# kocurvik/mdrp

Hardware: AMD Instinct MI355X
Metric: image-pairs/sec (2000 corrs, 10k RANSAC iters) (higher is better)
Workload: dtype f64

## Files before the change

mdrp_amd/build.py:

```python
import hashlib
import os
import re
import shutil
import subprocess

HERE = os.path.dirname(os.path.abspath(__file__))
SRC = os.path.join(HERE, "csrc", "mdrp_capi.hip")
SRC_TU = os.path.join(HERE, "csrc", "mdrp_tu.hip")
TU_GROUPS = (1, 2, 3)
DEPS = [SRC, SRC_TU, os.path.join(HERE, "csrc", "mdrp_kernels.h"), os.path.join(HERE, "csrc", "mdrp_math.h"),
        os.path.join(HERE, "csrc", "mdrp_classic.h"), os.path.join(HERE, "csrc", "mdrp_classic_math.h"),
        os.path.join(HERE, "csrc", "mdrp_logtab.h"), os.path.join(HERE, "csrc", "mdrp_instances.h"),
        os.path.join(HERE, "..", "include", "mdrp.h")]
OUT = os.path.join(HERE, "libmdrp_hip.so")
_MARK = b"MDRP_SRC_HASH="
FLAGS = ["-O3", "-std=c++17", "--offload-arch=gfx950", "-fPIC", "-shared", "-ffp-contract=fast", "-no-hip-rt"]


def hipcc():
    for c in (shutil.which("hipcc"), "/opt/rocm/bin/hipcc"):
        if c and os.path.exists(c):
            return c
    raise RuntimeError("hipcc not found")


def source_hash():
    h = hashlib.sha256()
    h.update(" ".join(FLAGS).encode())
    for d in DEPS:
        h.update(os.path.basename(d).encode() + b"\0")
        with open(d, "rb") as f:
            h.update(f.read())
    return h.hexdigest()[:16]


def built_hash(path=OUT):
    try:
        with open(path, "rb") as f:
            m = re.search(_MARK + rb"([0-9a-f]{16})", f.read())
        return m.group(1).decode() if m else None
    except OSError:
        return None


def up_to_date():
    return built_hash() == source_hash()


def build(force=False, verbose=False, defines=(), out=OUT, extra_flags=(), single=None):
    if not force and not defines and not extra_flags and out == OUT and up_to_date():
        return out
    if single is None:
        single = bool(defines) or bool(extra_flags)
    common = [*FLAGS, *extra_flags, f'-DMDRP_SRC_HASH="{source_hash()}"', *[f"-D{d}" for d in defines]]
    if verbose:
        common.insert(0, "-Rpass-analysis=kernel-resource-usage")
    if single:
        subprocess.check_call([hipcc(), *common, SRC, "-o", out + ".tmp"])
        os.replace(out + ".tmp", out)
        return out
    import tempfile
    from concurrent.futures import ThreadPoolExecutor
# ... 26 lines not shown
```

mdrp_amd/csrc/mdrp_capi.hip:

```cpp
#include "../../include/mdrp.h"
#include "mdrp_kernels.h"
#include "mdrp_classic.h"
#ifdef MDRP_SPLIT_TU
#define MDRP_INST extern
#include "mdrp_instances.h"
namespace mdrp {
MDRP_INSTANCES_FINAL_64
MDRP_INSTANCES_FINAL_256
MDRP_INSTANCES_CLASSIC
}
#endif

#include <algorithm>
#include <cmath>
#include <cstdio>
#include <cstdlib>
#include <cstddef>
#include <cstring>
#include <functional>
#include <map>
#include <mutex>
#include <string>
#include <vector>

using namespace mdrp;

static_assert(sizeof(mdrp_model) == sizeof(Model), "model layout");
static_assert(sizeof(mdrp_camera) == sizeof(CamDev), "camera layout");
static_assert(sizeof(mdrp_result) == sizeof(ResultDev), "result layout");

namespace {

thread_local std::string g_err;

#define HIPCHK(expr)                                                                                       \
    do {                                                                                                   \
        hipError_t e_ = (expr);                                                                            \
        if (e_ != hipSuccess) {                                                                            \
            char buf_[512];                                                                                \
            snprintf(buf_, sizeof buf_, "%s failed: %s (%s:%d)", #expr, hipGetErrorString(e_), __FILE__, __LINE__); \
            g_err = buf_;                                                                                  \
            return MDRP_ERR_HIP;                                                                           \
        }                                                                                                  \
    } while (0)

struct DevBuf {
    void *p = nullptr;
    size_t cap = 0;
    int ensure(size_t bytes) {
        if (bytes <= cap) return MDRP_OK;
        if (p) { (void)hipFree(p); p = nullptr; cap = 0; }
        size_t want = bytes + bytes / 8 + 256;
        hipError_t e = hipMalloc(&p, want);
        if (e != hipSuccess) { g_err = std::string("hipMalloc failed: ") + hipGetErrorString(e); p = nullptr; return MDRP_ERR_HIP; }
        cap = want;
        return MDRP_OK;
    }
    void release() { if (p) (void)hipFree(p); p = nullptr; cap = 0; }
    template <typename T> T *as() const { return reinterpret_cast<T *>(p); }
};

struct Progress {
// ... 432 lines not shown
            int rc_;
            if ((rc_ = get_events(h, &e0, &e1, 0))) return rc_;
            unsigned long long *cstats = reinterpret_cast<unsigned long long *>(cnt + 6);
            {
                hipEvent_t c0, c1;
                if ((rc_ = get_events(h, &c0, &c1, 1))) return rc_;
                const bool two_phase = !(it0 == 0 && c == 0);
                unsigned long long *cand_stat = h->cand_stat.as<unsigned long long>() + 2 * (size_t)p0;
                uint32_t *tags_u = tags_sc;
                int32_t *und_part = reinterpret_cast<int32_t *>((odd ? h->tags_s : h->tags2_s).as<uint32_t>() + so), *und_cnt = h->und_count.as<int32_t>() + 2 * (size_t)p0;
                const uint4 *rfrag_p = h->rfrag.as<uint4>() + (size_t)p0 * groups_max * 64;
                hipLaunchKernelGGL(k_count_plan, dim3(1), dim3(PLAN_THREADS), 0, s, pc, st_p, mcount_c, 2, CNT_WG_MODELS, h->cplan.as<int32_t>(),
                                   surv1, (const int32_t *)nullptr, two_phase ? und_cnt : (int32_t *)nullptr);
                const dim3 cgrid((unsigned)pc * (unsigned)((len * mps + CNT_WG_MODELS - 1) / CNT_WG_MODELS));
                HIPCHK(hipEventRecord(c0, s));
                MDRP_SWEEP_DISPATCH(k_count, kind, cgrid, dim3(CNT_THREADS), 0, s, r, st_p, rfrag_p, models_p,
                                    tags_c, mcount_c, h->cplan.as<int32_t>(), tags_v, surv1, cstats, (int32_t *)nullptr, (const int32_t *)nullptr,
                                    1, tags_u, und_part, und_cnt, (const int32_t *)nullptr, cand_stat);
                if (two_phase) {
                    hipLaunchKernelGGL(k_count_plan, dim3(1), dim3(PLAN_THREADS), 0, s, pc, st_p, und_cnt, 2, CNT_WG_MODELS, h->cplan.as<int32_t>(),
                                       (int32_t *)nullptr, (const int32_t *)nullptr, (int32_t *)nullptr);
                    MDRP_SWEEP_DISPATCH(k_count, kind, cgrid, dim3(CNT_THREADS), 0, s, r, st_p, rfrag_p, models_p,
                                        tags_u, und_cnt, h->cplan.as<int32_t>(), tags_v, surv1, cstats, (int32_t *)nullptr, (const int32_t *)nullptr,
                                        2, (uint32_t *)nullptr, (int32_t *)nullptr, (int32_t *)nullptr, und_part, cand_stat);
                    h->count_launches++;
                }
                HIPCHK(hipEventRecord(c1, s));
                h->count_launches++;
            }
            const uint32_t *surv_tags = tags_v;
            const int32_t *surv_cnt = surv1;
            if (use_bound && batch_call > 16 && !(it0 == 0 && c == 0)) {
                hipLaunchKernelGGL(k_count_plan, dim3(1), dim3(PLAN_THREADS), 0, s, pc, st_p, surv1, 1, BND_THREADS, h->cplan.as<int32_t>(), surv2, (const int32_t *)nullptr);
                const dim3 bgrid((unsigned)pc * (unsigned)((len * mps + BND_THREADS - 1) / BND_THREADS));
                unsigned long long *bstats = reinterpret_cast<unsigned long long *>(cnt + 12);
                hipEvent_t b0, b1;
                if ((rc_ = get_events(h, &b0, &b1, 4))) return rc_;
                HIPCHK(hipEventRecord(b0, s));
                MDRP_SWEEP_DISPATCH(k_bound, kind, bgrid, dim3(BND_THREADS), 0, s, r, st_p, pts_p, models_p, tags_v, surv1, h->cplan.as<int32_t>(), tags_c, surv2, bstats);
                HIPCHK(hipEventRecord(b1, s));
                surv_tags = tags_c; surv_cnt = surv2;
            }
            int32_t *plan = h->plan.as<int32_t>(), *totals = plan + 2 * (size_t)batch + 2;
            if (batch_call <= SCORE_WAVE_MAX_PAIRS) {
                hipLaunchKernelGGL(k_count_plan, dim3(1), dim3(PLAN_THREADS), 0, s, pc, st_p, surv_cnt, 1, SCW_THREADS / 64, plan, (int32_t *)nullptr, (const int32_t *)nullptr, (int32_t *)nullptr);
                hipLaunchKernelGGL(k_sort_tags, dim3(pc), dim3(256), 0, s, r, st_p, mcount_c, surv_cnt, surv_tags, tags_sc);
                HIPCHK(hipEventRecord(e0, s));
                const long long ub = (long long)pc * ((len * mps + SCW_THREADS / 64 - 1) / (SCW_THREADS / 64));
                const dim3 grid((unsigned)std::min<long long>(ub, (long long)h->num_cu * 32));
                MDRP_SWEEP_DISPATCH(k_score_w, kind, grid, dim3(SCW_THREADS), 0, s, r, st_p, pts_p, models_p, tags_sc, mcount_c,
                                    h->slot_score.as<double>() + so, h->slot_inl.as<int32_t>() + so, plan);
            } else {
                hipLaunchKernelGGL(k_sort_tags, dim3(pc), dim3(256), 0, s, r, st_p, mcount_c, surv_cnt, surv_tags, tags_sc);
                hipLaunchKernelGGL(k_plan, dim3(1), dim3(PLAN_THREADS), 0, s, pc, mcount_c, plan, totals);
                HIPCHK(hipEventRecord(e0, s));
                const dim3 grid((unsigned)pc * (unsigned)((len * mps + SCORE_THREADS - 1) / SCORE_THREADS));
                MDRP_SWEEP_DISPATCH(k_score, kind, grid, dim3(SCORE_THREADS), tile_bytes, s, r, st_p, pts_p, models_p, tags_sc, mcount_c,
                                    h->slot_score.as<double>() + so, h->slot_inl.as<int32_t>() + so, plan, totals);
            }
            HIPCHK(hipEventRecord(e1, s));
            h->sweep_launches++;
            Trigger *trig_p = h->triggers.as<Trigger>() + (size_t)p0 * trig_cap;
            unsigned long long *scan_stats = reinterpret_cast<unsigned long long *>(cnt + 10);
#define MDRP_SCAN(M, I) hipLaunchKernelGGL((k_scan<M, I>), dim3(pc), dim3(64), 0, s, r, st_p, h->slot_score.as<double>() + so, h->slot_inl.as<int32_t>() + so, trig_p, trig_cap, mcount_c, scan_stats)
            if (mps == 16) MDRP_SCAN(16, 1);
            else if (mps == 12) MDRP_SCAN(12, 1);
            else if (len >= 1024) MDRP_SCAN(4, 4);
            else MDRP_SCAN(4, 1);
#undef MDRP_SCAN
            return MDRP_OK;
        };
        bool solved1 = false;
        int swept0 = 0;
        if (host && it0 == 0) {
            const bool sliced = piped && n_chunks >= 2 && batch >= 2 * HOST_SLICE_PAIRS;
            const int sl = sliced ? HOST_SLICE_PAIRS : batch;
            for (int p0 = 0; p0 < batch; p0 += sl) {
                const int pc = std::min(sl, batch - p0);
                const size_t o2 = (size_t)2 * p0 * n_max, o1 = (size_t)p0 * n_max, n2 = sizeof(double) * 2 * (size_t)pc * n_max, n1 = sizeof(double) * (size_t)pc * n_max;
                hipStream_t cs = sliced ? h->copy_stream : s;
                HIPCHK(hipMemcpyAsync(const_cast<double *>(x1) + o2, host->x1 + o2, n2, hipMemcpyHostToDevice, cs));
                HIPCHK(hipMemcpyAsync(const_cast<double *>(x2) + o2, host->x2 + o2, n2, hipMemcpyHostToDevice, cs));
                if (host->d1 && host->d2) {
                    HIPCHK(hipMemcpyAsync(const_cast<double *>(d1) + o1, host->d1 + o1, n1, hipMemcpyHostToDevice, cs));
                    HIPCHK(hipMemcpyAsync(const_cast<double *>(d2) + o1, host->d2 + o1, n1, hipMemcpyHostToDevice, cs));
                }
                if (!sliced) { launch_prep(p0, pc, s); break; }
                HIPCHK(hipEventRecord(h->ev_copied, cs)); HIPCHK(hipStreamWaitEvent(aux, h->ev_copied, 0));
                if (p0 == 0) HIPCHK(hipStreamWaitEvent(aux, h->ev_tables, 0));
                launch_prep(p0, pc, aux);
                HIPCHK(hipEventRecord(h->ev_prepped, aux));
                if ((rc = issue_solve(1, aux, p0, pc))) return rc;
                const bool last = p0 + sl >= batch, last_but_one = !last && p0 + 2 * sl >= batch;
                if (last_but_one || last) HIPCHK(hipStreamWaitEvent(s, h->ev_prepped, 0));
                if (last_but_one) { swept0 = p0 + pc; if ((rc = issue_solve(0, s, 0, swept0)) || (rc = sweep_chunk(0, 0, swept0))) return rc; }
                if (last) { if ((rc = issue_solve(0, s, swept0, batch - swept0)) || (rc = sweep_chunk(0, swept0, batch - swept0))) return rc; swept0 = batch; }
            }
            if (sliced) { HIPCHK(hipEventRecord(h->ev_solved[1], aux)); solved1 = true; }
        }
        if (swept0 < batch && (rc = issue_solve(0, s, 0, batch))) return rc;
        if (piped) HIPCHK(hipEventRecord(h->ev_solved[0], s));
        for (int c = 0; c < n_chunks; ++c) {
            rp.chunk_len = (int)lens[c]; rp.chunk_off = offs[c];
            if (c == 0 && swept0 >= batch) {
                if (piped) HIPCHK(hipEventRecord(h->ev_scanned[0], s));
                continue;
            }
            if (piped && c + 1 < n_chunks && !(c == 0 && solved1)) {
                HIPCHK(hipStreamWaitEvent(aux, c == 0 ? h->ev_solved[0] : h->ev_scanned[c - 1], 0));
                if ((rc = issue_solve(c + 1, aux, 0, batch))) return rc;
                HIPCHK(hipEventRecord(h->ev_solved[c + 1], aux));
// ... 452 lines not shown
    HIPCHK(hipMemcpyAsync(out, h->unit_e.p, sizeof(Model) * M * count, hipMemcpyDeviceToHost, s));
    HIPCHK(hipMemcpyAsync(n_out, h->unit_f.p, sizeof(int32_t) * count, hipMemcpyDeviceToHost, s));
    HIPCHK(hipStreamSynchronize(s));
    return MDRP_OK;
}

int mdrp_score_models(mdrp_handle *h, int kind, int mem_space, const mdrp_model *models, int num_models, const double *x1,
                      const double *x2, int n, double sq_threshold, double *scores, int32_t *counts) {
    if (!h || num_models < 0 || n < 0 || kind < 0 || kind > 5 || !scores || !counts) { g_err = "invalid argument"; return MDRP_ERR_INVALID; }
    if (num_models == 0) return MDRP_OK;
    MDRP_ENTER(h);
    hipStream_t s = h->stream;
    const int chunk = (num_models + 3) / 4;
    const size_t slots = (size_t)chunk * 4;
    int rc;
    if ((rc = h->pts.ensure(sizeof(double) * PT_STRIDE * std::max(n, 1))) || (rc = h->st.ensure(sizeof(PairState))) ||
        (rc = h->models.ensure(sizeof(Model) * slots)) || (rc = h->slot_score.ensure(sizeof(double) * slots)) ||
        (rc = h->slot_inl.ensure(sizeof(int32_t) * slots)) || (rc = h->tags.ensure(sizeof(uint32_t) * slots)) ||
        (rc = h->model_count.ensure(2 * sizeof(int32_t))))
        return rc;
    const double *x1d = x1, *x2d = x2;
    const Model *md = reinterpret_cast<const Model *>(models);
    if (mem_space == MDRP_MEM_HOST) {
        if ((rc = h->in_x1.ensure(sizeof(double) * 2 * std::max(n, 1))) || (rc = h->in_x2.ensure(sizeof(double) * 2 * std::max(n, 1)))) return rc;
        HIPCHK(hipMemcpyAsync(h->in_x1.p, x1, sizeof(double) * 2 * n, hipMemcpyHostToDevice, s));
        HIPCHK(hipMemcpyAsync(h->in_x2.p, x2, sizeof(double) * 2 * n, hipMemcpyHostToDevice, s));
        HIPCHK(hipMemcpyAsync(h->models.p, models, sizeof(Model) * num_models, hipMemcpyHostToDevice, s));
        x1d = h->in_x1.as<double>(); x2d = h->in_x2.as<double>();
        md = h->models.as<Model>();
    } else {
        HIPCHK(hipMemcpyAsync(h->models.p, models, sizeof(Model) * num_models, hipMemcpyDeviceToDevice, s));
        md = h->models.as<Model>();
    }
    std::vector<uint32_t> tags(num_models);
    for (int i = 0; i < num_models; ++i) tags[i] = (uint32_t)i;
    HIPCHK(hipMemcpyAsync(h->tags.p, tags.data(), sizeof(uint32_t) * num_models, hipMemcpyHostToDevice, s));
    const int32_t counts2[2] = {num_models, 0};
    HIPCHK(hipMemcpyAsync(h->model_count.p, counts2, 2 * sizeof(int32_t), hipMemcpyHostToDevice, s));
    PairState ps;
    std::memset(&ps, 0, sizeof ps);
    ps.n = n; ps.active = 1; ps.sq_thr = sq_threshold; ps.eps = std::sqrt(sq_threshold);
    ps.best_min_score = DBL_MAX;
    HIPCHK(hipMemcpyAsync(h->st.p, &ps, sizeof ps, hipMemcpyHostToDevice, s));
    hipLaunchKernelGGL(k_pack_unit, dim3((n + 255) / 256 + 1), dim3(256), 0, s, n, x1d, x2d, (const double *)nullptr,
                       (const double *)nullptr, h->pts.as<double>(), (double *)nullptr);
    hipLaunchKernelGGL(k_box_unit, dim3(1), dim3(256), 0, s, n, h->pts.as<double>(), h->st.as<PairState>());
    RunParams rp;
    std::memset(&rp, 0, sizeof rp);
    rp.kind = kind; rp.batch = 1; rp.n_max = std::max(n, 1); rp.chunk_len = chunk; rp.chunk_off = 0; rp.slot_stride = chunk * 4; rp.super_len = chunk;
    rp.mps = 4; rp.sample_sz = 3;
    const size_t tile_bytes = SCORE_TILE_BYTES;
    if ((rc = h->plan.ensure(sizeof(int32_t) * 8))) return rc;
    int32_t *plan = h->plan.as<int32_t>(), *totals = plan + 4;
    hipLaunchKernelGGL(k_plan, dim3(1), dim3(PLAN_THREADS), 0, s, 1, h->model_count.as<int32_t>(), plan, totals);
    const dim3 grid((unsigned)std::min(h->num_cu * 4, (num_models + SCORE_THREADS - 1) / SCORE_THREADS));
    h->ev_used = 0; h->sweep_launches = 1; h->sweep_evals = (int64_t)num_models * n;
    hipEvent_t e0, e1;
    if ((rc = get_events(h, &e0, &e1))) return rc;
    HIPCHK(hipEventRecord(e0, s));
    MDRP_SWEEP_DISPATCH(k_score, kind, grid, dim3(SCORE_THREADS), tile_bytes, s, rp, h->st.as<PairState>(), h->pts.as<double>(), md,
                        h->tags.as<uint32_t>(), h->model_count.as<int32_t>(), h->slot_score.as<double>(), h->slot_inl.as<int32_t>(), plan, totals);
    HIPCHK(hipEventRecord(e1, s));
    HIPCHK(hipGetLastError());
    const hipMemcpyKind back = mem_space == MDRP_MEM_HOST ? hipMemcpyDeviceToHost : hipMemcpyDeviceToDevice;
    HIPCHK(hipMemcpyAsync(scores, h->slot_score.p, sizeof(double) * num_models, back, s));
    HIPCHK(hipMemcpyAsync(counts, h->slot_inl.p, sizeof(int32_t) * num_models, back, s));
    return finish_timing(h);
}

int mdrp_count_candidates(mdrp_handle *h, int kind, const mdrp_model *models, int num_models, const double *x1, const double *x2,
                          int n, double sq_threshold, int32_t *candidates) {
    if (!h || num_models < 0 || n < 0 || kind < 0 || kind > 5 || !candidates || !models) { g_err = "invalid argument"; return MDRP_ERR_INVALID; }
    if (num_models == 0) return MDRP_OK;
    MDRP_ENTER(h);
    hipStream_t s = h->stream;
    const int nn = std::max(n, 1);
    const size_t slots = (size_t)num_models;
    int rc;
    if ((rc = h->pts.ensure(sizeof(double) * PT_STRIDE * nn)) || (rc = h->st.ensure(sizeof(PairState))) ||
        (rc = h->models.ensure(sizeof(Model) * slots)) || (rc = h->slot_inl.ensure(sizeof(int32_t) * slots)) ||
        (rc = h->tags.ensure(sizeof(uint32_t) * slots)) || (rc = h->tags_v.ensure(sizeof(uint32_t) * slots)) ||
        (rc = h->model_count.ensure(2 * sizeof(int32_t))) || (rc = h->surv_count.ensure(sizeof(int32_t))) ||
        (rc = h->cplan.ensure(2 * sizeof(int32_t))) || (rc = h->rfrag.ensure((size_t)((nn + 15) / 16) * 1024)) ||
        (rc = h->unit_f.ensure(sizeof(int32_t) * slots)) || (rc = h->in_x1.ensure(sizeof(double) * 2 * nn)) ||
        (rc = h->in_x2.ensure(sizeof(double) * 2 * nn)))
        return rc;
    HIPCHK(hipMemcpyAsync(h->in_x1.p, x1, sizeof(double) * 2 * n, hipMemcpyHostToDevice, s));
    HIPCHK(hipMemcpyAsync(h->in_x2.p, x2, sizeof(double) * 2 * n, hipMemcpyHostToDevice, s));
    HIPCHK(hipMemcpyAsync(h->models.p, models, sizeof(Model) * num_models, hipMemcpyHostToDevice, s));
    std::vector<uint32_t> tags(num_models);
    for (int i = 0; i < num_models; ++i) tags[i] = (uint32_t)i;
    HIPCHK(hipMemcpyAsync(h->tags.p, tags.data(), sizeof(uint32_t) * num_models, hipMemcpyHostToDevice, s));
    const int32_t counts2[2] = {num_models, 0};
    HIPCHK(hipMemcpyAsync(h->model_count.p, counts2, 2 * sizeof(int32_t), hipMemcpyHostToDevice, s));
    HIPCHK(hipMemsetAsync(h->surv_count.p, 0, sizeof(int32_t), s));
    PairState ps;
    std::memset(&ps, 0, sizeof ps);
    ps.n = n; ps.active = 1; ps.sq_thr = sq_threshold; ps.eps = std::sqrt(sq_threshold);
    ps.best_min_score = DBL_MAX;
    HIPCHK(hipMemcpyAsync(h->st.p, &ps, sizeof ps, hipMemcpyHostToDevice, s));
    hipLaunchKernelGGL(k_pack_unit, dim3((n + 255) / 256 + 1), dim3(256), 0, s, n, h->in_x1.as<double>(), h->in_x2.as<double>(),
                       (const double *)nullptr, (const double *)nullptr, h->pts.as<double>(), (double *)nullptr);
    hipLaunchKernelGGL(k_box_unit, dim3(1), dim3(256), 0, s, n, h->pts.as<double>(), h->st.as<PairState>());
    hipLaunchKernelGGL(k_frag_unit, dim3((n + 16 + 255) / 256), dim3(256), 0, s, n, h->pts.as<double>(), h->rfrag.as<uint4>());
    RunParams rp;
    std::memset(&rp, 0, sizeof rp);
    rp.kind = kind; rp.batch = 1; rp.n_max = nn; rp.slot_stride = num_models; rp.mps = 4; rp.sample_sz = 3;
// ... 121 lines not shown
```

mdrp_amd/csrc/mdrp_instances.h:

```cpp
#pragma once
namespace mdrp {
#define MDRP_FINAL_PARAMS RunParams, PairState *, const double *, const double *, uint8_t *, ResultDev *, int, int, unsigned long long *, const int32_t *, int32_t *, \
                          unsigned long long, unsigned long long *
#define MDRP_FINAL_LOSSES(X, K, S, T) X(K, S, T, 0) X(K, S, T, 1) X(K, S, T, 2) X(K, S, T, 3) X(K, S, T, 4) X(K, S, T, 5)
#define MDRP_FINAL_KINDS(X, T) MDRP_FINAL_LOSSES(X, 0, false, T) MDRP_FINAL_LOSSES(X, 0, true, T) MDRP_FINAL_LOSSES(X, 1, false, T) MDRP_FINAL_LOSSES(X, 2, false, T)
#define MDRP_FINAL_ONE(K, S, T, L) MDRP_INST template __global__ void k_final<K, S, T, L>(MDRP_FINAL_PARAMS);

#define MDRP_CLASSIC_KINDS_T(X, T) X(CLASSIC_RELPOSE, T) X(CLASSIC_SHARED, T) X(CLASSIC_FUND, T)
#define MDRP_KC_LO_ONE(CK, T) MDRP_INST template __global__ void kc_lo<CK, T>(RunParams, const PairState *, const double *, const Model *, Trigger *, int, const int32_t *, int32_t *, \
                                                                               int32_t *, uint8_t *, int, FuseTail);
#define MDRP_KC_FINAL_ONE(CK, T) MDRP_INST template __global__ void kc_final<CK, T>(RunParams, PairState *, const double *, uint8_t *, ResultDev *, const int32_t *, int32_t *, \
                                                                                     unsigned long long, unsigned long long *, int);
#define MDRP_KC_REFINE_ONE(CK, T) MDRP_INST template __global__ void kc_refine_unit<CK, T>(int, Model *, const double *, int, LmOpt, double *);
#define MDRP_KC_SOLVE_ONE(CK) MDRP_INST template __global__ void kc_solve<CK>(RunParams, const PairState *, const uint32_t *, const double *, Model *, int32_t *, uint32_t *, int32_t *);
#define MDRP_KC_UNIT_ONE(CK) MDRP_INST template __global__ void kc_solver_unit<CK>(int, const double *, const double *, Model *, int32_t *);
#define MDRP_KC_SAMPLES_ONE(K) MDRP_INST template __global__ void kc_samples<K>(int, const int32_t *, uint64_t *, int, uint32_t *);

#define MDRP_INSTANCES_FINAL_64 MDRP_FINAL_KINDS(MDRP_FINAL_ONE, 64)
#define MDRP_INSTANCES_FINAL_256 MDRP_FINAL_KINDS(MDRP_FINAL_ONE, 256)
#define MDRP_INSTANCES_CLASSIC                                                                                                       \
    MDRP_CLASSIC_KINDS_T(MDRP_KC_LO_ONE, 64) MDRP_CLASSIC_KINDS_T(MDRP_KC_LO_ONE, 256)                                              \
    MDRP_CLASSIC_KINDS_T(MDRP_KC_FINAL_ONE, 64) MDRP_CLASSIC_KINDS_T(MDRP_KC_FINAL_ONE, 256)                                        \
    MDRP_CLASSIC_KINDS_T(MDRP_KC_REFINE_ONE, 64) MDRP_CLASSIC_KINDS_T(MDRP_KC_REFINE_ONE, 256)                                      \
    MDRP_KC_SOLVE_ONE(CLASSIC_SHARED) MDRP_KC_SOLVE_ONE(CLASSIC_FUND)  \
    MDRP_KC_UNIT_ONE(CLASSIC_RELPOSE) MDRP_KC_UNIT_ONE(CLASSIC_SHARED) MDRP_KC_UNIT_ONE(CLASSIC_FUND)                               \
    MDRP_KC_SAMPLES_ONE(5) MDRP_KC_SAMPLES_ONE(6) MDRP_KC_SAMPLES_ONE(7)
}
```

mdrp_amd/csrc/mdrp_kernels.h:

```cpp
#pragma once
#include <hip/hip_runtime.h>
#include <float.h>
#include "mdrp_logtab.h"
#include "mdrp_math.h"

#ifdef MDRP_SECONDARY_TU
#define MDRP_GLOBAL static __global__
#else
#define MDRP_GLOBAL __global__
#endif

namespace mdrp {

constexpr int PT_STRIDE = 6;
#define MDRP_TILE_PTS 512
#define MDRP_SCORE_MINWAVES 4
constexpr int TILE_PTS = MDRP_TILE_PTS;
constexpr size_t SCORE_TILE_BYTES = (size_t)TILE_PTS * (PT_STRIDE * sizeof(double) + 4 * sizeof(float));
#define MDRP_P1F_UNROLL 8
#define MDRP_P1_UNROLL 4
constexpr int PRUNE_EVERY = 4;
#define MDRP_DENSE_KEY 40
#define MDRP_SOLVE_MINWAVES 2
#define MDRP_SCORE_THREADS 256
// ... 1114 lines not shown
    const unsigned long long ball = __ballot(surv);
    if (ball) {
        int base = 0;
        const int first = __ffsll((long long)ball) - 1;
        if (lane == first) base = atomicAdd(&cnt_out[pair], __popcll(ball));
        base = __shfl(base, first, 64);
        if (surv) tags_out[slot_base + base + __popcll(ball & ((1ull << lane) - 1ull))] = tag;
    }
    if (stats && tid == 0 && blk == 0) atomicAdd(stats, (unsigned long long)cnt * (unsigned long long)n);
}

MDRP_GLOBAL __launch_bounds__(256) void k_sort_tags(RunParams rp, const PairState *__restrict__ st, int32_t *__restrict__ model_count,
                                                   const int32_t *__restrict__ surv_count,
                                                   const uint32_t *__restrict__ tags, uint32_t *__restrict__ tags_sorted) {
    const int pair = blockIdx.x, tid = threadIdx.x;
    const PairState &ps = st[pair];
    if (!ps.active) return;
    __shared__ int s_hist[PROBE_PTS + 1], s_pos[PROBE_PTS + 1];
    __shared__ int s_dense;
    if (tid <= PROBE_PTS) s_hist[tid] = 0;
    if (tid == 0) s_dense = 0;
    __syncthreads();
    const int cnt = surv_count[pair];
    const size_t slot_base = (size_t)pair * rp.slot_stride;
    const uint32_t *src = tags + slot_base;
    uint32_t *dst = tags_sorted + slot_base;
    const int dense_min = ps.n >= 8 ? MDRP_DENSE_KEY : PROBE_PTS + 1;
    for (int i = tid; i < cnt; i += 256) atomicAdd(&s_hist[min(src[i] >> 24, (uint32_t)PROBE_PTS)], 1);
    __syncthreads();
    if (tid < 64) {
        const int v = tid < dense_min ? s_hist[tid] : 0;
        int incl = v;
#pragma unroll
        for (int o = 1; o < 64; o <<= 1) {
            const int u = __shfl_up(incl, o, 64);
            if (tid >= o) incl += u;
        }
        s_pos[tid] = incl - v;
        if (tid == 63) s_pos[64] = incl;
    }
    __syncthreads();
    const int cap = rp.slot_stride;
    for (int i = tid; i < cnt; i += 256) {
        const uint32_t t = src[i];
        const int key = (int)min(t >> 24, (uint32_t)PROBE_PTS);
        if (key >= dense_min) dst[cap - 1 - atomicAdd(&s_dense, 1)] = t & 0xFFFFFFu;
        else dst[atomicAdd(&s_pos[key], 1)] = t & 0xFFFFFFu;
    }
    __syncthreads();
    if (tid == 0) { model_count[2 * pair] = cnt - s_dense; model_count[2 * pair + 1] = s_dense; }
}

MDRP_GLOBAL __launch_bounds__(PLAN_THREADS) void k_plan(int batch, const int32_t *__restrict__ model_count, int32_t *__restrict__ plan,
                                                       int32_t *__restrict__ totals ) {
    __shared__ int s_w[PLAN_THREADS / 64 + 1];
    int run_d = 0, run_s = 0;
    int32_t *pd = plan, *psp = plan + batch + 1;
    for (int p0 = 0; p0 < batch; p0 += PLAN_THREADS) {
        const int p = p0 + threadIdx.x;
        int bd = 0, bs = 0;
        if (p < batch) {
            bs = (model_count[2 * p] + SCORE_THREADS - 1) / SCORE_THREADS;
            bd = (model_count[2 * p + 1] + SCORE_THREADS - 1) / SCORE_THREADS;
        }
        int tot_d, tot_s;
        const int ed = plan_block_scan(bd, tot_d, s_w), es = plan_block_scan(bs, tot_s, s_w);
        if (p < batch) { pd[p] = run_d + run_s + ed + es; psp[p] = bs; }
        run_d += tot_d;
        run_s += tot_s;
    }
    if (threadIdx.x == 0) { pd[batch] = run_d + run_s; psp[batch] = 0; totals[0] = run_d; totals[1] = run_d + run_s; totals[2] = 0; }
}

template <bool POSE, bool RAWF = false>
__global__ __launch_bounds__(SCORE_THREADS, MDRP_SCORE_MINWAVES) void k_score(RunParams rp, const PairState *__restrict__ st, const double *__restrict__ pts,
                                                         const Model *__restrict__ models, const uint32_t *__restrict__ tags,
                                                         const int32_t *__restrict__ model_count, double *__restrict__ slot_score,
                                                         int32_t *__restrict__ slot_inl, const int32_t *__restrict__ plan,
                                                         int32_t *__restrict__ totals) {
    extern __shared__ double tile[];
    float4 *tile32 = reinterpret_cast<float4 *>(tile + TILE_PTS * PT_STRIDE);
    const int total = totals[1];
    const int tid = threadIdx.x;
    for (int w = blockIdx.x; w < total; w += gridDim.x) {
    const int pair = plan_find(plan, rp.batch, w);
    const int blk_sparse = plan[rp.batch + 1 + pair];
    const int bi = w - plan[pair];
    const bool dense = bi >= blk_sparse;
    const int blk = dense ? bi - blk_sparse : bi;
    const int cnt_sparse = model_count[2 * pair], cnt_dense = model_count[2 * pair + 1];
    const PairState &ps = st[pair];
    const int n = ps.n;
    const double thr = ps.sq_thr;
    const size_t slot_base = (size_t)pair * rp.slot_stride;
    const int cap = rp.slot_stride;
    bool live;
    uint32_t slot = 0;
    {
        const int i = blk * SCORE_THREADS + tid;
        live = i < (dense ? cnt_dense : cnt_sparse);
        if (live) slot = tags[slot_base + (dense ? cap - 1 - i : i)];
    }
    double E[9], thr_dmax;
    float tb, Ef[9];
    const Model *mp = models + slot_base + slot;
#pragma unroll
    for (int i = 0; i < 9; ++i) E[i] = 0;
    if (live) {
        const Model m = *mp;
        double R[9], Em[9];
        if (RAWF) {
#pragma unroll
            for (int i = 0; i < 9; ++i) E[i] = reinterpret_cast<const double *>(&m)[i];
        } else {
            quat_to_R(m.q, R);
            essential_from_Rt(R, m.t, Em);
// ... 55 lines not shown
        const int i = (w - plan[pair]) * (SCW_THREADS / 64) + wave;
        const int cnt_sparse = model_count[2 * pair], cnt_dense = model_count[2 * pair + 1];
        if (i >= cnt_sparse + cnt_dense) continue;
        const PairState &ps = st[pair];
        const int n = ps.n;
        const double thr = ps.sq_thr;
        const size_t slot_base = (size_t)pair * rp.slot_stride;
        const uint32_t slot = tags[slot_base + (i < cnt_sparse ? i : rp.slot_stride - 1 - (i - cnt_sparse))];
        const Model m = models[slot_base + slot];
        double E[9], R[9], t[3] = {m.t[0], m.t[1], m.t[2]};
#pragma unroll
        for (int q = 0; q < 9; ++q) R[q] = 0;
        if (RAWF) {
#pragma unroll
            for (int q = 0; q < 9; ++q) E[q] = reinterpret_cast<const double *>(&m)[q];
        } else {
            double Em[9];
            quat_to_R(m.q, R);
            essential_from_Rt(R, m.t, Em);
            if (POSE) {
#pragma unroll
                for (int q = 0; q < 9; ++q) E[q] = Em[q];
            } else fundamental_from_E(Em, m.f1, m.f2, E);
        }
        const long long rec_cnt = (long long)ps.best_min_cnt;
        const double rec_score = ps.best_min_score < DBL_MAX ? ps.best_min_score * (1.0 + 1e-12) : DBL_MAX;
        const double *gp = pts + (size_t)pair * rp.n_max * PT_STRIDE;
        double score = 0;
        int cnt = 0;
        bool pruned = false;
        for (int t0 = 0; t0 < n; t0 += 64) {
            const int r = t0 + lane;
            double s1 = 0;
            int c1 = 0;
            if (r < n) score_point<POSE>(gp + (size_t)r * PT_STRIDE, E, R, t, thr, s1, c1);
            const unsigned long long ball = __ballot(c1 != 0);
            if (ball) {
                if (c1) s_r2[wave][__popcll(ball & lt)] = s1;
                __builtin_amdgcn_fence(__ATOMIC_RELEASE, "wavefront");
                __builtin_amdgcn_wave_barrier();
                __builtin_amdgcn_fence(__ATOMIC_ACQUIRE, "wavefront");
                const int k = __popcll(ball);
                for (int j = 0; j < k; ++j) score += s_r2[wave][j];
                cnt += k;
                __builtin_amdgcn_wave_barrier();
            }
            const int processed = min(t0 + 64, n);
            if (rec_score < DBL_MAX && ((processed & 127) == 0 || processed == n) &&
                (long long)cnt + (long long)(n - processed) <= rec_cnt && score + thr * (double)(processed - cnt) >= rec_score) { pruned = true; break; }
        }
        if (lane == 0) {
            slot_score[slot_base + slot] = pruned ? DBL_MAX : score + thr * (double)(n - cnt);
            slot_inl[slot_base + slot] = pruned ? -2 : cnt;
        }
    }
}

template <int MPS = 4, int IPL = 1>
__global__ __launch_bounds__(64) void k_scan(RunParams rp, PairState *__restrict__ st, const double *__restrict__ slot_score,
                                             const int32_t *__restrict__ slot_inl, Trigger *__restrict__ triggers,
                                             int trig_cap, const int32_t *__restrict__ model_count,
                                             unsigned long long *__restrict__ evals) {
    const int pair = blockIdx.x, lane = threadIdx.x;
    PairState &ps = st[pair];
    if (!ps.active) { if (lane == 0) ps.n_triggers = 0; return; }
    if (lane == 0 && evals) atomicAdd(evals, (unsigned long long)(model_count[2 * pair] + model_count[2 * pair + 1]) * (unsigned long long)ps.n);
    long long run_cnt = (long long)ps.best_min_cnt;
    double run_score = ps.best_min_score;
    const double nan_score = (double)ps.n * ps.sq_thr;
    int ntrig = rp.chunk_off > 0 ? ps.n_triggers : 0;
    static_assert(MPS % 4 == 0, "slots of an iteration are read as 16-byte groups");
    constexpr int NG = MPS / 4;
    const size_t slot_base = (size_t)pair * rp.slot_stride + (size_t)rp.chunk_off * MPS;
    struct Slots { int4 c[IPL][NG]; double2 s01[IPL][NG], s23[IPL][NG]; };
    auto fetch = [&](int it0) {
        Slots r;
#pragma unroll
        for (int j = 0; j < IPL; ++j) {
            const int it = it0 + IPL * lane + j;
#pragma unroll
            for (int g = 0; g < NG; ++g) {
                if (it < rp.chunk_len) {
                    r.c[j][g] = *reinterpret_cast<const int4 *>(slot_inl + slot_base + (size_t)it * MPS + 4 * g);
                    const double2 *sp = reinterpret_cast<const double2 *>(slot_score + slot_base + (size_t)it * MPS + 4 * g);
                    r.s01[j][g] = sp[0]; r.s23[j][g] = sp[1];
                } else { r.c[j][g] = make_int4(-1, -1, -1, -1); r.s01[j][g] = r.s23[j][g] = make_double2(DBL_MAX, DBL_MAX); }
            }
        }
        return r;
    };
    Slots nxt = fetch(0);
    for (int it0 = 0; it0 < rp.chunk_len; it0 += 64 * IPL) {
        const Slots cur = nxt;
        if (it0 + 64 * IPL < rp.chunk_len) nxt = fetch(it0 + 64 * IPL);
        int c[IPL][MPS];
        double s[IPL][MPS];
        long long lc = -1;
        double ls = DBL_MAX;
#pragma unroll
        for (int j = 0; j < IPL; ++j) {
#pragma unroll
            for (int g = 0; g < NG; ++g) {
                c[j][4 * g] = cur.c[j][g].x; c[j][4 * g + 1] = cur.c[j][g].y; c[j][4 * g + 2] = cur.c[j][g].z; c[j][4 * g + 3] = cur.c[j][g].w;
                s[j][4 * g] = c[j][4 * g] >= 0 ? cur.s01[j][g].x : DBL_MAX; s[j][4 * g + 1] = c[j][4 * g + 1] >= 0 ? cur.s01[j][g].y : DBL_MAX;
                s[j][4 * g + 2] = c[j][4 * g + 2] >= 0 ? cur.s23[j][g].x : DBL_MAX; s[j][4 * g + 3] = c[j][4 * g + 3] >= 0 ? cur.s23[j][g].y : DBL_MAX;
            }
// ... 853 lines not shown
```

mdrp_amd/csrc/mdrp_tu.hip:

```cpp
#define MDRP_SECONDARY_TU 1
#include "mdrp_kernels.h"
#include "mdrp_classic.h"
#define MDRP_INST
#include "mdrp_instances.h"
namespace mdrp {
#if MDRP_TU == 1
MDRP_INSTANCES_FINAL_64
#elif MDRP_TU == 2
MDRP_INSTANCES_FINAL_256
#elif MDRP_TU == 3
MDRP_INSTANCES_CLASSIC
#else
#error "MDRP_TU must be 1 (k_final, 64 lanes), 2 (k_final, 256 lanes) or 3 (5- / 6- / 7-point baselines)"
#endif
}
```

Before: 126,200.

## Add split scoring kernel with producer/consumer wavefronts for later RANSAC chunks

Adds k_score_split, where each 320-thread block scores 64 hypotheses. Four wavefronts evaluate 8-point slices of a shared-memory point tile and write residuals and inlier bitmasks into double-buffered LDS. A fifth wavefront accumulates scores and decides early termination per hypothesis. The launch uses a persistent grid capped at 16 blocks per CU and is used for every sweep except the first chunk of the first iteration. k_plan is generalized to take per-item block size and class flags. The aim is to spread each hypothesis's point loop across several wavefronts and share point loads, at the cost of extra block barriers per 32-point step and a serialized reduction wave.

After: 128,100 (median of 6 runs). 1.01x the previous value.

```diff
diff --git a/mdrp_amd/build.py b/mdrp_amd/build.py
--- a/mdrp_amd/build.py
+++ b/mdrp_amd/build.py
@@ -7,7 +7,7 @@
 HERE = os.path.dirname(os.path.abspath(__file__))
 SRC = os.path.join(HERE, "csrc", "mdrp_capi.hip")
 SRC_TU = os.path.join(HERE, "csrc", "mdrp_tu.hip")
-TU_GROUPS = (1, 2, 3)
+TU_GROUPS = (1, 2, 3, 4)
 DEPS = [SRC, SRC_TU, os.path.join(HERE, "csrc", "mdrp_kernels.h"), os.path.join(HERE, "csrc", "mdrp_math.h"),
         os.path.join(HERE, "csrc", "mdrp_classic.h"), os.path.join(HERE, "csrc", "mdrp_classic_math.h"),
         os.path.join(HERE, "csrc", "mdrp_logtab.h"), os.path.join(HERE, "csrc", "mdrp_instances.h"),
diff --git a/mdrp_amd/csrc/mdrp_capi.hip b/mdrp_amd/csrc/mdrp_capi.hip
--- a/mdrp_amd/csrc/mdrp_capi.hip
+++ b/mdrp_amd/csrc/mdrp_capi.hip
@@ -8,6 +8,7 @@
 MDRP_INSTANCES_FINAL_64
 MDRP_INSTANCES_FINAL_256
 MDRP_INSTANCES_CLASSIC
+MDRP_INSTANCES_SCORE
 }
 #endif
 
@@ -546,11 +547,20 @@
                                     h->slot_score.as<double>() + so, h->slot_inl.as<int32_t>() + so, plan);
             } else {
                 hipLaunchKernelGGL(k_sort_tags, dim3(pc), dim3(256), 0, s, r, st_p, mcount_c, surv_cnt, surv_tags, tags_sc);
-                hipLaunchKernelGGL(k_plan, dim3(1), dim3(PLAN_THREADS), 0, s, pc, mcount_c, plan, totals);
-                HIPCHK(hipEventRecord(e0, s));
                 const dim3 grid((unsigned)pc * (unsigned)((len * mps + SCORE_THREADS - 1) / SCORE_THREADS));
-                MDRP_SWEEP_DISPATCH(k_score, kind, grid, dim3(SCORE_THREADS), tile_bytes, s, r, st_p, pts_p, models_p, tags_sc, mcount_c,
-                                    h->slot_score.as<double>() + so, h->slot_inl.as<int32_t>() + so, plan, totals);
+                if (it0 == 0 && c == 0) {
+                    hipLaunchKernelGGL(k_plan, dim3(1), dim3(PLAN_THREADS), 0, s, pc, mcount_c, plan, totals, SCORE_THREADS, 3);
+                    HIPCHK(hipEventRecord(e0, s));
+                    MDRP_SWEEP_DISPATCH(k_score, kind, grid, dim3(SCORE_THREADS), tile_bytes, s, r, st_p, pts_p, models_p, tags_sc, mcount_c,
+                                        h->slot_score.as<double>() + so, h->slot_inl.as<int32_t>() + so, plan, totals);
+                } else {
+                    hipLaunchKernelGGL(k_plan, dim3(1), dim3(PLAN_THREADS), 0, s, pc, mcount_c, plan, totals, SCX_HYPS, 3);
+                    HIPCHK(hipEventRecord(e0, s));
+                    const long long ub = (long long)pc * ((len * mps + SCX_HYPS - 1) / SCX_HYPS);
+                    const dim3 xgrid((unsigned)std::min<long long>(ub, (long long)h->num_cu * 16));
+                    MDRP_SWEEP_DISPATCH(k_score_split, kind, xgrid, dim3(SCX_THREADS), 0, s, r, st_p, pts_p, models_p, tags_sc, mcount_c,
+                                        h->slot_score.as<double>() + so, h->slot_inl.as<int32_t>() + so, plan, totals);
+                }
             }
             HIPCHK(hipEventRecord(e1, s));
             h->sweep_launches++;
@@ -1109,7 +1119,7 @@
     const size_t tile_bytes = SCORE_TILE_BYTES;
     if ((rc = h->plan.ensure(sizeof(int32_t) * 8))) return rc;
     int32_t *plan = h->plan.as<int32_t>(), *totals = plan + 4;
-    hipLaunchKernelGGL(k_plan, dim3(1), dim3(PLAN_THREADS), 0, s, 1, h->model_count.as<int32_t>(), plan, totals);
+    hipLaunchKernelGGL(k_plan, dim3(1), dim3(PLAN_THREADS), 0, s, 1, h->model_count.as<int32_t>(), plan, totals, SCORE_THREADS, 3);
     const dim3 grid((unsigned)std::min(h->num_cu * 4, (num_models + SCORE_THREADS - 1) / SCORE_THREADS));
     h->ev_used = 0; h->sweep_launches = 1; h->sweep_evals = (int64_t)num_models * n;
     hipEvent_t e0, e1;
diff --git a/mdrp_amd/csrc/mdrp_instances.h b/mdrp_amd/csrc/mdrp_instances.h
--- a/mdrp_amd/csrc/mdrp_instances.h
+++ b/mdrp_amd/csrc/mdrp_instances.h
@@ -25,4 +25,7 @@
     MDRP_KC_SOLVE_ONE(CLASSIC_SHARED) MDRP_KC_SOLVE_ONE(CLASSIC_FUND)  \
     MDRP_KC_UNIT_ONE(CLASSIC_RELPOSE) MDRP_KC_UNIT_ONE(CLASSIC_SHARED) MDRP_KC_UNIT_ONE(CLASSIC_FUND)                               \
     MDRP_KC_SAMPLES_ONE(5) MDRP_KC_SAMPLES_ONE(6) MDRP_KC_SAMPLES_ONE(7)
+#define MDRP_SCORE_SPLIT_ONE(P, R) MDRP_INST template __global__ void k_score_split<P, R>(RunParams, const PairState *, const double *, const Model *, const uint32_t *, \
+                                                                                      const int32_t *, double *, int32_t *, const int32_t *, const int32_t *);
+#define MDRP_INSTANCES_SCORE MDRP_SCORE_SPLIT_ONE(true, false) MDRP_SCORE_SPLIT_ONE(false, false) MDRP_SCORE_SPLIT_ONE(false, true)
 }
diff --git a/mdrp_amd/csrc/mdrp_kernels.h b/mdrp_amd/csrc/mdrp_kernels.h
--- a/mdrp_amd/csrc/mdrp_kernels.h
+++ b/mdrp_amd/csrc/mdrp_kernels.h
@@ -1190,7 +1190,7 @@
 }
 
 MDRP_GLOBAL __launch_bounds__(PLAN_THREADS) void k_plan(int batch, const int32_t *__restrict__ model_count, int32_t *__restrict__ plan,
-                                                       int32_t *__restrict__ totals ) {
+                                                       int32_t *__restrict__ totals , int per_item, int classes) {
     __shared__ int s_w[PLAN_THREADS / 64 + 1];
     int run_d = 0, run_s = 0;
     int32_t *pd = plan, *psp = plan + batch + 1;
@@ -1198,8 +1198,8 @@
         const int p = p0 + threadIdx.x;
         int bd = 0, bs = 0;
         if (p < batch) {
-            bs = (model_count[2 * p] + SCORE_THREADS - 1) / SCORE_THREADS;
-            bd = (model_count[2 * p + 1] + SCORE_THREADS - 1) / SCORE_THREADS;
+            bs = (classes & 1) ? (model_count[2 * p] + per_item - 1) / per_item : 0;
+            bd = (classes & 2) ? (model_count[2 * p + 1] + per_item - 1) / per_item : 0;
         }
         int tot_d, tot_s;
         const int ed = plan_block_scan(bd, tot_d, s_w), es = plan_block_scan(bs, tot_s, s_w);
@@ -1361,6 +1361,126 @@
         if (lane == 0) {
             slot_score[slot_base + slot] = pruned ? DBL_MAX : score + thr * (double)(n - cnt);
             slot_inl[slot_base + slot] = pruned ? -2 : cnt;
+        }
+    }
+}
+
+constexpr int SCX_EVAL = 4;
+constexpr int SCX_THREADS = 64 * (SCX_EVAL + 1);
+constexpr int SCX_STEP = 32;
+constexpr int SCX_SLICE = SCX_STEP / SCX_EVAL;
+constexpr int SCX_TILE = 256;
+constexpr int SCX_HYPS = 64;
+static_assert(SCX_SLICE == 8 && SCX_TILE % SCX_STEP == 0, "an evaluating wavefront's slice is one byte of the step's inlier mask");
+template <bool POSE, bool RAWF = false>
+__global__ __launch_bounds__(SCX_THREADS) void k_score_split(RunParams rp, const PairState *__restrict__ st, const double *__restrict__ pts,
+                                                             const Model *__restrict__ models, const uint32_t *__restrict__ tags ,
+                                                             const int32_t *__restrict__ model_count, double *__restrict__ slot_score,
+                                                             int32_t *__restrict__ slot_inl, const int32_t *__restrict__ plan ,
+                                                             const int32_t *__restrict__ totals) {
+    __shared__ double s_rec[SCX_TILE * PT_STRIDE];
+    __shared__ double s_r2[2][SCX_STEP][SCX_HYPS];
+    __shared__ uint32_t s_inl[2][SCX_HYPS];
+    __shared__ unsigned long long s_dead[2];
+    const int total = totals[1];
+    const int lane = threadIdx.x & 63, wave = threadIdx.x >> 6;
+    for (int w = blockIdx.x; w < total; w += gridDim.x) {
+        const int pair = plan_find(plan, rp.batch, w);
+        const int blk_sparse = plan[rp.batch + 1 + pair];
+        const int bi = w - plan[pair];
+        const bool dense = bi >= blk_sparse;
+        const int blk = dense ? bi - blk_sparse : bi;
+        const int cnt_sparse = model_count[2 * pair], cnt_dense = model_count[2 * pair + 1];
+        const PairState &ps = st[pair];
+        const int n = ps.n;
+        const double thr = ps.sq_thr;
+        const size_t slot_base = (size_t)pair * rp.slot_stride;
+        const int cap = rp.slot_stride;
+        const int i = blk * SCX_HYPS + lane;
+        const bool live = i < (dense ? cnt_dense : cnt_sparse);
+        const uint32_t slot = live ? tags[slot_base + (dense ? cap - 1 - i : i)] : 0u;
+        double E[9], R[9], t[3] = {0, 0, 0};
+#pragma unroll
+        for (int q = 0; q < 9; ++q) E[q] = R[q] = 0;
+        if (live && wave != 0) {
+            const Model m = models[slot_base + slot];
+            if (RAWF) {
+#pragma unroll
+                for (int q = 0; q < 9; ++q) E[q] = reinterpret_cast<const double *>(&m)[q];
+            } else {
+                double Em[9];
+                quat_to_R(m.q, R);
+                essential_from_Rt(R, m.t, Em);
+                if (POSE) {
+#pragma unroll
+                    for (int q = 0; q < 9; ++q) E[q] = Em[q];
+                    t[0] = m.t[0]; t[1] = m.t[1]; t[2] = m.t[2];
+                } else {
+                    fundamental_from_E(Em, m.f1, m.f2, E);
+                }
+            }
+        }
+        const long long rec_cnt = (long long)ps.best_min_cnt;
+        const double rec_score = ps.best_min_score < DBL_MAX ? ps.best_min_score * (1.0 + 1e-12) : DBL_MAX;
+        double score = 0;
+        int cnt = 0;
+        bool dead = !live;
+        __syncthreads();
+        if (wave == 0) {
+            const unsigned long long d0 = __ballot(dead);
+            if (lane == 0) { s_dead[0] = d0; s_dead[1] = d0; }
+        }
+        const double *gp = pts + (size_t)pair * rp.n_max * PT_STRIDE;
+        const int nsteps = (n + SCX_STEP - 1) / SCX_STEP;
+        for (int k = 0; k <= nsteps; ++k) {
+            __syncthreads();
+            const unsigned long long dmask = s_dead[k & 1];
+            if (dmask == ~0ull) break;
+            const int r0 = k * SCX_STEP;
+            if (k < nsteps && r0 % SCX_TILE == 0) {
+                const int npts = min(SCX_TILE, n - r0);
+                const double2 *src = reinterpret_cast<const double2 *>(gp + (size_t)r0 * PT_STRIDE);
+                double2 *dst = reinterpret_cast<double2 *>(s_rec);
+                for (int j = threadIdx.x; j < npts; j += SCX_THREADS) {
+                    const double2 p0 = src[3 * j], p1 = src[3 * j + 1], p2 = src[3 * j + 2];
+                    dst[3 * j] = p0; dst[3 * j + 1] = p1; dst[3 * j + 2] = p2;
+                }
+                __syncthreads();
+            }
+            if (wave == 0) {
+                if (k > 0) {
+                    const int b = (k - 1) & 1, q0 = r0 - SCX_STEP, g = min(SCX_STEP, n - q0);
+                    const uint32_t m = s_inl[b][lane];
+                    for (int j = 0; j < g; ++j) score += s_r2[b][j][lane];
+                    cnt += __popc(m);
+                    if (rec_score < DBL_MAX) {
+                        const int processed = q0 + g;
+                        dead = dead || (((long long)cnt + (long long)(n - processed) <= rec_cnt) && (score + thr * (double)(processed - cnt) >= rec_score));
+                        const unsigned long long d = __ballot(dead);
+                        if (lane == 0) s_dead[b] = d;
+                    }
+                }
+            } else if (k < nsteps) {
+                const int e = wave - 1, b = k & 1;
+                const int q = r0 + e * SCX_SLICE, g = min(SCX_SLICE, n - q), tq = q % SCX_TILE;
+                uint32_t inl = 0;
+                if (g > 0 && !((dmask >> lane) & 1ull)) {
+                    const double *base = s_rec + (size_t)tq * PT_STRIDE;
+                    double *out = &s_r2[b][e * SCX_SLICE][lane];
+                    for (int j = 0; j < g; ++j) {
+                        double s1 = 0;
+                        int c1 = 0;
+                        score_point<POSE>(base + j * PT_STRIDE, E, R, t, thr, s1, c1);
+                        out[j * SCX_HYPS] = s1;
+                        inl |= (uint32_t)c1 << j;
+                    }
+                }
+                reinterpret_cast<uint8_t *>(&s_inl[b][lane])[e] = (uint8_t)inl;
+            }
+        }
+        if (wave == 0 && live) {
+            slot_score[slot_base + slot] = dead ? DBL_MAX : score + thr * (double)(n - cnt);
+            slot_inl[slot_base + slot] = dead ? -2 : cnt;
         }
     }
 }
diff --git a/mdrp_amd/csrc/mdrp_tu.hip b/mdrp_amd/csrc/mdrp_tu.hip
--- a/mdrp_amd/csrc/mdrp_tu.hip
+++ b/mdrp_amd/csrc/mdrp_tu.hip
@@ -10,7 +10,9 @@
 MDRP_INSTANCES_FINAL_256
 #elif MDRP_TU == 3
 MDRP_INSTANCES_CLASSIC
+#elif MDRP_TU == 4
+MDRP_INSTANCES_SCORE
 #else
-#error "MDRP_TU must be 1 (k_final, 64 lanes), 2 (k_final, 256 lanes) or 3 (5- / 6- / 7-point baselines)"
+#error "MDRP_TU must be 1 (k_final, 64 lanes), 2 (k_final, 256 lanes), 3 (5- / 6- / 7-point baselines) or 4 (k_score_split)"
 #endif
 }
```
